# lisanhu/LongReadMapper

Hardware: AMD Instinct MI355X
Metric: aligned Gbp/sec (higher is better)
Workload: dtype u8/u64 integer; 1 GPU; E. coli K-12 sized synthetic reference (4641652 bp, 5% planted repeats), 100000 x 10000 bp ont-profile reads per GPU; seed_len=20, thres=300, gact_T=320, gact_O=120, gact_W=128, reads_per_gpu=100000, read_len=10000, streams=3, sa_sampled=1, parallelism=reads sharded, index replicated (1 RCCL bcast)

## Files before the change

### longreadmapper_amd/csrc/index_tables.hip

```cpp
#include <hip/hip_runtime.h>
#include <cstdio>
#include "seed_index_dev.h"

__device__ __forceinline__ uint64_t lcl_entry(const LrmIndexView &ix, int hl, uint64_t code) {
    const int ext = hl - ix.hlen;
    uint64_t k, l;
    lc_lookup(ix, code >> (2 * ext), k, l);
    if (k == 0 && l == 0) return 0;
    for (int i = ext - 1; i >= 0 && k <= l; --i) {
        const uint32_t c = (uint32_t) (code >> (2 * i)) & 3u;
        uint64_t ra, rb;
        occ_lf2(ix, c, k - 1, l, ra, rb);
        k = ra + 1;
        l = rb;
    }
    if (k > l) return 0;
    const uint64_t cnt = l - k + 1;
    return cnt >= 0xFFFFFFull ? (0xFFFFFFull << 40) : (k | (cnt << 40));
}

__global__ __launch_bounds__(256) void lcl_build_kernel(LrmIndexView ix, int hl, int pair, int kbits, uint64_t *__restrict__ out,
                                                        uint64_t slot0, uint64_t *__restrict__ ovf, uint64_t ovf_cap,
                                                        unsigned long long *__restrict__ n_ovf) {
    const uint64_t slot = slot0 + (uint64_t) blockIdx.x * 256 + threadIdx.x;
// ... 92 lines not shown
    }
    bool to_side = rr >= cmax;
    for (uint32_t r = 0; r < (uint32_t) sdv.sd_f; ++r) {
        const SdKey key = sd_key_of(sdv, code, r);
        uint64_t *line = sd + key.line * 8;
        bool placed = false;
        if (sdv.sd_slot == 8) {
            const uint64_t v = k | (c << sdv.sd_kbits) | (key.tag << (64u - key.tb));
            for (int sl = 0; sl < 8 && !placed; ++sl)
                placed = atomicCAS((unsigned long long *) &line[sl], 0ull, (unsigned long long) v) == 0ull;
            if (!placed) atomicOr((unsigned long long *) &line[0], 1ull << (63u - key.tb));
        } else {
            const uint64_t v = k | (c << sdv.sd_kbits) | (key.tag << (48u - key.tb));
            const uint32_t at = atomicAdd(reinterpret_cast<uint32_t *>(line) + 15, 1u) & 0xFFu;
            if (at >= 250u) atomicAdd(n_ovf, 1ull << 40);
            if (at >= 10u) atomicOr(reinterpret_cast<uint32_t *>(line) + 15, 1u << (8u + sd_filter_bit((uint32_t) key.tag)));
            if (at < 10u) {
                uint16_t *h = reinterpret_cast<uint16_t *>(line) + 3 * at;
                h[0] = (uint16_t) v; h[1] = (uint16_t) (v >> 16); h[2] = (uint16_t) (v >> 32);
                placed = true;
            }
        }
        if (!placed) to_side = true;
    }
    if (to_side) {
        const unsigned long long at = atomicAdd(n_ovf, 1ull);
        if (at < ovf_cap) { ovf[2 * at] = code; ovf[2 * at + 1] = side; }
    }
}

__global__ __launch_bounds__(256) void sd_clear_kernel(ulonglong2 *__restrict__ p, uint64_t n16) {
    for (uint64_t i = (uint64_t) blockIdx.x * 256 + threadIdx.x; i < n16; i += (uint64_t) gridDim.x * 256) p[i] = make_ulonglong2(0, 0);
}

struct SdPlan { int f, bits, slot, kbits, cbits; uint64_t bytes; };
static bool sd_plan(const lrm_index *idx, uint64_t free_b, SdPlan *pl) {
    const LrmIndexTune &tu = idx->itune;
    const uint64_t L = idx->view.length;
    const int S = tu.sd_len;
    if (tu.sd == 0 || !idx->cpl_ok || L < 64 || idx->view.con_len != L) return false;
    int kbits = 1;
    while ((1ull << kbits) < L) ++kbits;
    for (int f = 4; f >= 2; f -= 2) {
        if (tu.sd_f && tu.sd_f != f) continue;
        const int slot = f == 4 ? 8 : 6, lf = f == 4 ? 2 : 1;
        const double target = f == 4 ? 2.2 : 6.0;
        int bits = 10;
        while ((double) f * (double) L / (double) (1ull << bits) > target && bits < 34) ++bits;
        if (tu.sd_bits) bits = tu.sd_bits;
        const int CL2 = 2 * (S - f + 1);
        if (bits > CL2) bits = CL2;
        if (bits < 11) bits = 11;
        if (bits < CL2 - 31) bits = CL2 - 31;
        const int tb = lf + 2 * (f - 1) + (CL2 - bits);
        int cbits = (slot == 8 ? 63 : 48) - tb - kbits;
        if (cbits < (tu.sd_bits ? 2 : 4) || tb > 40) continue;
        if (cbits > 24) cbits = 24;
        if (tu.sd_cbits && tu.sd_cbits < cbits) cbits = tu.sd_cbits;
        const uint64_t bytes = 64ull << bits;
        const uint64_t spare = bytes >= (32ull << 30) ? (40ull << 30) : (8ull << 30);
        if (tu.sd < 0 && ((uint64_t) free_b < bytes + bytes / 8 + spare || (tu.lc_long_max >= 13 && bytes > (16ull << 30)))) continue;
        pl->f = f; pl->bits = bits; pl->slot = slot; pl->kbits = kbits; pl->cbits = cbits; pl->bytes = bytes;
        return true;
    }
    return false;
}
static void sd_filter_build(lrm_index *idx);
static int sd_build(lrm_index *idx, const SdPlan &pl) {
    uint64_t *d = nullptr, *ovf = nullptr, *tab = nullptr;
    uint32_t *claimed = nullptr;
    unsigned long long *n_ovf = nullptr;
    const char *why = "";
    unsigned long long n = 0;
    auto give_up = [&]() {
        if (idx->mtune.verbose) fprintf(stderr, "[lrm] seed table (share %d, 2^%d lines, %d-byte slots) not built: %s (side entries %llu)\n", pl.f, pl.bits, pl.slot, why, n);
        if (d) (void) hipFree(d); if (ovf) (void) hipFree(ovf); if (tab) (void) hipFree(tab); if (n_ovf) (void) hipFree(n_ovf);
        if (claimed) (void) hipFree(claimed);
        (void) hipGetLastError(); return 0; };
    const uint64_t L = idx->view.length, lines = 1ull << pl.bits;
    uint64_t ovf_cap = lines / 4 + 4096;
    if (ovf_cap > (1ull << 30)) ovf_cap = 1ull << 30;
    if (idx->itune.sd_bits) ovf_cap = (uint64_t) pl.f * L + 4096;
    why = "no room for the table";
    if (hipMalloc(&d, pl.bytes) != hipSuccess) { d = nullptr; return give_up(); }
    why = "no room for the overflow list";
    if (hipMalloc(&ovf, ovf_cap * 16) != hipSuccess) { ovf = nullptr; return give_up(); }
    if (hipMalloc(&n_ovf, 8) != hipSuccess) { n_ovf = nullptr; return give_up(); }
    const uint64_t cl_bytes = ((L + 31) / 32 + 1) * 4;
    if (hipMalloc(&claimed, cl_bytes) != hipSuccess) { claimed = nullptr; return give_up(); }
    why = "memset failed";
    if (hipMemset(claimed, 0, cl_bytes) != hipSuccess) return give_up();
    hipLaunchKernelGGL(sd_clear_kernel, dim3(256 * 64), dim3(256), 0, 0, reinterpret_cast<ulonglong2 *>(d), pl.bytes / 16);
    if (hipGetLastError() != hipSuccess || hipMemset(n_ovf, 0, 8) != hipSuccess) return give_up();
    LrmIndexView sdv = idx->view;
    sdv.sd_len = idx->itune.sd_len; sdv.sd_f = pl.f; sdv.sd_bits = pl.bits; sdv.sd_kbits = pl.kbits; sdv.sd_slot = pl.slot; sdv.sd_cbits = pl.cbits;
    const uint64_t chunk = 1ull << 22;
    for (uint64_t b0 = 0, blocks = (L + 255) / 256; b0 < blocks; b0 += chunk) {
        const uint64_t nb = blocks - b0 < chunk ? blocks - b0 : chunk;
        hipLaunchKernelGGL(sd_build_kernel, dim3((uint32_t) nb), dim3(256), 0, 0, idx->view, sdv, d, b0 * 256, claimed, ovf, ovf_cap, n_ovf);
    }
    why = "build kernel failed";
    if (hipDeviceSynchronize() != hipSuccess) { give_up(); lrm_set_error("seed table build failed"); return -1; }
    why = "too many entries beside their lines";
    if (hipMemcpy(&n, n_ovf, 8, hipMemcpyDeviceToHost) != hipSuccess || n > ovf_cap) return give_up();
    uint64_t tslots = 1024;
    while (tslots < 2 * n) tslots <<= 1;
    why = "no room for the side table";
    if (hipMalloc(&tab, tslots * 16) != hipSuccess) { tab = nullptr; return give_up(); }
    if (hipMemset(tab, 0, tslots * 16) != hipSuccess) return give_up();
    if (n) hipLaunchKernelGGL(lclx_build_kernel, dim3((uint32_t) ((n + 255) / 256)), dim3(256), 0, 0, ovf, (uint64_t) n, tab, tslots - 1);
    if (hipDeviceSynchronize() != hipSuccess) { give_up(); lrm_set_error("seed table side build failed"); return -1; }
    (void) hipFree(ovf); (void) hipFree(n_ovf); (void) hipFree(claimed);
    idx->d_sd = d; idx->d_sdx = tab;
    idx->view.sd = d; idx->view.sdx = tab; idx->view.sdx_mask = tslots - 1;
    idx->view.sd_len = sdv.sd_len; idx->view.sd_f = pl.f; idx->view.sd_bits = pl.bits; idx->view.sd_kbits = pl.kbits; idx->view.sd_slot = pl.slot;
    idx->view.sd_cbits = pl.cbits;
    idx->sd_side_entries = n;
    if (idx->mtune.verbose) fprintf(stderr, "[lrm] seed table: %d positions per line, 2^%d lines, %d-byte slots, %d count bits, %llu side entries\n", pl.f, pl.bits, pl.slot, pl.cbits, n);
    sd_filter_build(idx);
    return 0;
}

__global__ __launch_bounds__(256) void sd_filter_kernel(const ulonglong2 *__restrict__ sd, uint64_t lines, uint32_t g,
                                                        uint32_t *__restrict__ filt) {
    const uint64_t line = (uint64_t) blockIdx.x * 256 + threadIdx.x;
    if (line >= lines) return;
    const ulonglong2 x0 = sd[line * 4], x1 = sd[line * 4 + 1], x2 = sd[line * 4 + 2], x3 = sd[line * 4 + 3];
    if (((x0.x | x0.y) | (x1.x | x1.y) | (x2.x | x2.y) | (x3.x | x3.y)) == 0) return;
    const uint64_t bit = line >> g;
    const uint32_t m = 1u << (bit & 31u);
    if (!(filt[bit >> 5] & m)) atomicOr(&filt[bit >> 5], m);
}
__global__ __launch_bounds__(256) void sd_filter_count_kernel(const uint32_t *__restrict__ filt, uint64_t words,
                                                              unsigned long long *__restrict__ n_set) {
    uint32_t c = 0;
    for (uint64_t i = (uint64_t) blockIdx.x * 256 + threadIdx.x; i < words; i += (uint64_t) gridDim.x * 256) c += __popc(filt[i]);
    for (int o = 32; o > 0; o >>= 1) c += __shfl_down(c, o, 64);
    if ((threadIdx.x & 63u) == 0 && c) atomicAdd(n_set, (unsigned long long) c);
}
static void sd_filter_build(lrm_index *idx) {
    const LrmIndexView &v = idx->view;
    const int kb = idx->itune.sd_filter_kb;
    if (kb <= 0 || !lrm_sd48_form(v)) return;
    const uint64_t lines = 1ull << v.sd_bits, max_bits = (uint64_t) kb * 8192;
    uint32_t g = 0;
    while ((lines >> g) > max_bits) ++g;
    const uint64_t bits = lines >> g;
    if (bits < 512) return;
    if ((double) v.length / (double) bits > 4.0 * 0.6931471805599453) {
        if (idx->mtune.verbose) fprintf(stderr, "[lrm] seed filter: not built, %.1f rows per bit at %d KiB\n", (double) v.length / (double) bits, kb);
        return;
    }
    uint32_t *filt = nullptr;
    unsigned long long *d_n = nullptr, n_set = 0;
    bool ok = hipMalloc(&filt, bits / 8 + 64) == hipSuccess && hipMalloc(&d_n, 8) == hipSuccess
              && hipMemset(filt, 0, bits / 8 + 64) == hipSuccess && hipMemset(d_n, 0, 8) == hipSuccess;
    if (ok) {
        const uint64_t chunk = 1ull << 30;
        for (uint64_t l0 = 0; l0 < lines; l0 += chunk) {
            const uint64_t nl = lines - l0 < chunk ? lines - l0 : chunk;
            hipLaunchKernelGGL(sd_filter_kernel, dim3((uint32_t) ((nl + 255) / 256)), dim3(256), 0, 0,
                               reinterpret_cast<const ulonglong2 *>(v.sd) + l0 * 4, nl, g, filt + ((l0 >> g) >> 5));
        }
        hipLaunchKernelGGL(sd_filter_count_kernel, dim3(256), dim3(256), 0, 0, filt, bits / 32, d_n);
        ok = hipDeviceSynchronize() == hipSuccess && hipMemcpy(&n_set, d_n, 8, hipMemcpyDeviceToHost) == hipSuccess;
    }
    if (d_n) (void) hipFree(d_n);
    const bool keep = ok && 2 * n_set <= bits;
    if (idx->mtune.verbose && ok)
        fprintf(stderr, "[lrm] seed filter: %llu bytes, one bit per %u lines, %.1f %% of the bits set%s\n", (unsigned long long) (bits / 8), 1u << g,
                100.0 * (double) n_set / (double) bits, keep ? "" : ": more than half, not kept");
    if (!keep) { if (filt) (void) hipFree(filt); (void) hipGetLastError(); return; }
    idx->d_sd_filt = filt;
    idx->view.sd_filt = filt; idx->view.sd_filt_shift = (int32_t) g;
}
// ... 91 lines not shown
```

### longreadmapper_amd/csrc/lrm_internal.h

```cpp
#pragma once
#include <stddef.h>
#include <stdint.h>
#include <stdlib.h>
#include <string.h>
#include "../../include/lrm_accel.h"

#define LRM_BLOB_MAGIC 0x4c524d424c4f4232ull
#define LRM_OCC_ROWS 64

struct LrmOccEntry {
    uint64_t cnt;
    uint64_t mask;
};
struct LrmOccBlock { LrmOccEntry sym[4]; };
static_assert(sizeof(LrmOccBlock) == 64, "occ block must be one 64-B line");

struct LrmMtaDev { uint64_t offset, seq_len; };

struct LrmBlobHeader {
    uint64_t magic, version;
    uint64_t length;
    uint64_t c4[4];
    uint64_t dollar_row;
    uint64_t n_blocks;
    uint64_t lc_entries;
    uint64_t sa_len, con_len;
    uint64_t off_occ, off_lc, off_sa, off_content, off_mta;
    uint64_t total_bytes;
    int32_t hlen, mta_len;
    uint64_t off_lcx, n_lcx;
    uint64_t sa_ratio;
    uint64_t reserved[10];
};
static_assert(sizeof(LrmBlobHeader) == 256, "header is 256 B");

struct LrmIndexView {
    const LrmOccBlock *occ;
    const uint64_t *lc;
    const uint64_t *lcx;
    uint64_t n_lcx;
    const uint64_t *sa;
    const char *content;
    const LrmMtaDev *mta;
    uint64_t length, dollar_row, sa_len, con_len;
    uint64_t c4[4];
    int32_t hlen, mta_len;
    const uint64_t *lcl;
    int32_t hl;
    int32_t sa_shift;
    int32_t lcl_pair;
    int32_t lcl_kbits;
    const uint64_t *core;
    const uint64_t *lclx;
    uint64_t lclx_mask;
    const uint64_t *sd;
    const uint64_t *sdx;
    uint64_t sdx_mask;
    int32_t sd_len;
    int32_t sd_f;
    int32_t sd_bits;
    int32_t sd_kbits;
    int32_t sd_slot;
    int32_t sd_cbits;
    const uint32_t *sd_filt;
    int32_t sd_filt_shift;
};
static inline bool lrm_sd48_form(const LrmIndexView &v) {
    return v.sd && v.sd_f == 4 && v.sd_slot == 8 && 8 + 2 * (v.sd_len - 3) - v.sd_bits <= 32;
}

struct LrmEnv {
    static constexpr int MAXV = 32;
    const char *name[MAXV];
    long long val[MAXV];
    int n;
    bool get(const char *key, long long *out) const;
};
void lrm_env_snapshot(LrmEnv *e);
#define LRM_SD_FILTER_KB_DEFAULT 4096
struct LrmIndexTune {
    int sa_ratio;
    int lc_long, lc_long_max, lc_pair, lc_entry_bytes, lc_count_bits, lc_core;
    int sd, sd_len, sd_f, sd_bits, sd_cbits;
    int sd_filter_kb;
    uint64_t lcx_threshold;
};
struct LrmMapTune {
    int dense, gact_impl, seed_rounds, cigar_text, keep_reads, anchored;
    uint32_t anchor_min_len;
    uint32_t clip, clip_penalty, clip_end_bonus;
    uint32_t split, split_min_len;
    uint32_t slice_reads, sub_batches, group_subs, bs_waves, copy_threads;
    uint32_t ss_items, ss_lds_pad, vote_vg, vote_t1, vote_u, vote_load, vote_fast;
    uint32_t t3_limit, t3_slots;
    int ext_streams, seed_streams, verbose;
};
void lrm_resolve_index_tune(const lrm_index_options *opt, const LrmEnv &env, LrmIndexTune *out);
void lrm_resolve_map_tune(const lrm_map_options *opt, const LrmEnv &env, LrmMapTune *out);
template <typename T>
static inline void lrm_options_over_defaults(T *o, const T *opt) {
    if (opt) memcpy(o, opt, opt->struct_size && opt->struct_size < sizeof(T) ? opt->struct_size : sizeof(T));
}
template <typename T>
static inline void lrm_options_take_fields(T *o, const T *opt, size_t from, size_t to) {
    if (opt && opt->struct_size >= to) memcpy((char *) o + from, (const char *) opt + from, to - from);
}

struct LrmHostCtx;
struct lrm_index;
void lrm_call_map_tune(const lrm_index *ix, const lrm_map_options *opt, LrmMapTune *out);
struct lrm_index {
    void *d_blob;
    uint64_t blob_bytes;
    int owns_blob;
    int device;
    LrmBlobHeader hdr;
    LrmIndexView view;
    uint64_t *d_lcl;
    uint64_t *d_lclx;
    uint64_t *d_core;
    uint64_t *d_sd, *d_sdx;
    uint64_t sd_side_entries;
    uint32_t *d_sd_filt;
    uint64_t *d_cpl;
    int cpl_ok;
    uint64_t *d_sas;
    LrmHostCtx *host;
    int n_peers;
    lrm_index **peers;
    LrmEnv env;
    LrmIndexTune itune;
    LrmMapTune mtune;
    uint32_t dbg_t3_limit, dbg_t3_slots;
    uint32_t dbg_mapq_slots;
};

struct LrmPhaseRes {
    uint64_t key1, val1, bucket1;
    uint64_t key2, val2, bucket2;
};

struct LrmDevCounters {
    unsigned long long bs_queue;
    unsigned long long vote_ticket[2];
    unsigned long long seed_traffic[3];
    unsigned long long reserved[2];
    unsigned long long decided_phase0;
    unsigned long long gact_tiles;
    unsigned long long pad[2];
    unsigned long long vote_fast_ticket[2];
    unsigned long long vote_redo_n[2];
    unsigned long long vote_big_n[2];
// ... 176 lines not shown
```

### longreadmapper_amd/csrc/seed_index_dev.h

```cpp
#pragma once
#include "lrm_hip_util.h"

__device__ __forceinline__ uint32_t base_code(uint32_t c) { return ((c >> 1) ^ (c >> 2)) & 3u; }

__device__ __forceinline__ uint32_t occ_lf2(const LrmIndexView &ix, uint32_t c, uint64_t loc_a, uint64_t loc_b,
                                            uint64_t &ra, uint64_t &rb) {
    const ulonglong2 eb = *reinterpret_cast<const ulonglong2 *>(&ix.occ[loc_b >> 6].sym[c]);
    ulonglong2 ea = eb;
    const bool two = (loc_a >> 6) != (loc_b >> 6);
    if (two) ea = *reinterpret_cast<const ulonglong2 *>(&ix.occ[loc_a >> 6].sym[c]);
    ra = occ_lf_of(ea, loc_a);
    rb = occ_lf_of(eb, loc_b);
    return two ? 2u : 1u;
}

__device__ __forceinline__ void lc_lookup(const LrmIndexView &ix, uint64_t code, uint64_t &k, uint64_t &l) {
    const uint64_t e = ix.lc[code];
    k = e & ((1ull << 40) - 1ull);
    const uint64_t cnt = e >> 40;
    l = k + cnt - 1;
    if (e == 0) { k = 0; l = 0; }
    else if (cnt == 0xFFFFFFull) {
        uint64_t lo = 0, hi = ix.n_lcx;
        while (lo < hi) { uint64_t mid = (lo + hi) >> 1; if (ix.lcx[3 * mid] < code) lo = mid + 1; else hi = mid; }
        k = ix.lcx[3 * lo + 1];
        l = ix.lcx[3 * lo + 2];
    }
}

struct SdKey { uint64_t line; uint64_t tag; uint32_t tb; };
__device__ __forceinline__ SdKey sd_key_of(const LrmIndexView &ix, uint64_t code, uint32_t r) {
    const uint32_t lf = ix.sd_f == 4 ? 2u : 1u, F = 1u << lf, lo_n = F - 1u - r;
    const uint32_t CL2 = 2u * ((uint32_t) ix.sd_len - F + 1u), wlo = CL2 < 32u ? CL2 : 32u;
    const uint64_t core = (code >> (2u * lo_n)) & ((1ull << CL2) - 1ull);
    const uint32_t extra = (uint32_t) (code & ((1ull << (2u * lo_n)) - 1ull)) | ((uint32_t) (code >> (2u * lo_n + CL2)) << (2u * lo_n));
    uint32_t m = (uint32_t) core * 0x9E3779B1u;
    if (wlo < 32u) m &= (1u << wlo) - 1u;
    const uint32_t chi = ((uint32_t) (core >> 32) ^ m) & ((1u << (CL2 - wlo)) - 1u);
    const uint32_t rb = CL2 - (uint32_t) ix.sd_bits;
    SdKey key;
    key.line = ((uint64_t) chi << (wlo - rb)) | (uint64_t) (m >> rb);
    key.tb = lf + 2u * (F - 1u) + rb;
    key.tag = (uint64_t) (r | (extra << lf)) | ((uint64_t) (m & ((1u << rb) - 1u)) << (lf + 2u * (F - 1u)));
    return key;
}
__device__ __forceinline__ uint32_t sd_filter_bit(uint32_t tag) { return (((tag * 0x9E3779B1u) >> 27) * 24u) >> 5; }
__device__ __forceinline__ bool sd_side_lookup(const LrmIndexView &ix, uint64_t code, uint64_t &e) {
    uint64_t slot = (code * 0x9E3779B97F4A7C15ull) >> 20 & ix.sdx_mask;
    for (;;) {
        const ulonglong2 x = *reinterpret_cast<const ulonglong2 *>(ix.sdx + 2 * slot);
        if (x.x == code + 1) { e = x.y; return true; }
        if (x.x == 0) return false;
        slot = (slot + 1) & ix.sdx_mask;
    }
}
__device__ __forceinline__ int sd_search(const LrmIndexView &ix, const SdKey &key, uint64_t code, const uint64_t (&W)[8],
                                         uint64_t &k, uint64_t &c, uint32_t *cnt) {
    uint64_t e = 0;
    bool ovf;
    if (ix.sd_slot == 8) {
        if (key.tb <= 32u) {
            const uint32_t sh = 32u - key.tb, t32 = (uint32_t) key.tag;
            uint32_t elo = 0, ehi = 0;
#pragma unroll
            for (int i = 7; i >= 0; --i) {
                const uint32_t hi = (uint32_t) (W[i] >> 32);
                const bool m = (hi >> sh) == t32;
                elo = m ? (uint32_t) W[i] : elo;
                ehi = m ? hi : ehi;
            }
            e = (uint64_t) elo | ((uint64_t) ehi << 32);
        } else {
#pragma unroll
            for (int i = 7; i >= 0; --i)
                if ((W[i] >> (64u - key.tb)) == key.tag) e = W[i];
        }
        ovf = (W[0] >> (63u - key.tb)) & 1ull;
    } else {
        uint32_t D[16];
#pragma unroll
        for (int i = 0; i < 8; ++i) { D[2 * i] = (uint32_t) W[i]; D[2 * i + 1] = (uint32_t) (W[i] >> 32); }
        if (key.tb <= 16u) {
            const uint32_t sh = 16u - key.tb, t32 = (uint32_t) key.tag;
            uint32_t elo = 0, ehi = 0;
#pragma unroll
            for (int i = 9; i >= 0; --i) {
                const int h2 = 3 * i + 2;
                const uint32_t hw = (h2 & 1) ? D[h2 >> 1] >> 16 : D[h2 >> 1] & 0xFFFFu;
                const uint32_t lo = (i & 1) ? __builtin_amdgcn_alignbit(D[(3 * i + 1) >> 1], D[(3 * i) >> 1], 16) : D[(3 * i) >> 1];
                const bool m = (hw >> sh) == t32;
                elo = m ? lo : elo;
                ehi = m ? hw : ehi;
            }
            e = (uint64_t) elo | ((uint64_t) ehi << 32);
        } else {
#pragma unroll
            for (int i = 9; i >= 0; --i) {
                const int w = (48 * i) >> 6, off = (48 * i) & 63;
                uint64_t v = W[w] >> off;
                if (off > 16) v |= W[w + 1] << (64 - off);
                v &= (1ull << 48) - 1ull;
                if ((v >> (48u - key.tb)) == key.tag) e = v;
            }
        }
        ovf = (D[15] & 0xFFu) > 10u && ((D[15] >> (8u + sd_filter_bit((uint32_t) key.tag))) & 1u);
    }
    const uint64_t cmax = (1ull << ix.sd_cbits) - 1ull;
    if (e != 0) {
        k = e & ((1ull << ix.sd_kbits) - 1ull);
        c = (e >> ix.sd_kbits) & cmax;
        if (c == 0) { k |= LRM_LOCATED_BIT; c = 1; return 1; }
        if (c != cmax) return 1;
    } else if (!ovf) {
        return 0;
    }
    uint64_t se;
    if (cnt) cnt[0] += 2;
    if (!sd_side_lookup(ix, code, se)) return e != 0 ? 2 : 0;
    if ((se >> 40) == 0xFFFFFFull) return 2;
    k = se & ((1ull << 40) - 1ull);
    c = se >> 40;
    return 1;
}
__device__ __forceinline__ int sd_lookup(const LrmIndexView &ix, uint64_t win, uint32_t jpar, uint64_t &k, uint64_t &c, uint32_t *cnt) {
    const uint64_t code = win & ((1ull << (2 * ix.sd_len)) - 1ull);
    const SdKey key = sd_key_of(ix, code, jpar & (uint32_t) (ix.sd_f - 1));
    const uint64_t *line = ix.sd + key.line * 8;
    const ulonglong2 x0 = *reinterpret_cast<const ulonglong2 *>(line), x1 = *reinterpret_cast<const ulonglong2 *>(line + 2);
    const ulonglong2 x2 = *reinterpret_cast<const ulonglong2 *>(line + 4), x3 = *reinterpret_cast<const ulonglong2 *>(line + 6);
    if (cnt) cnt[0] += 1;
    const uint64_t W[8] = {x0.x, x0.y, x1.x, x1.y, x2.x, x2.y, x3.x, x3.y};
    return sd_search(ix, key, code, W, k, c, cnt);
}

__device__ __forceinline__ uint64_t seed_one(const LrmIndexView &ix, uint64_t win, int seed_len, uint32_t jpar,
                                             uint64_t &k, uint64_t &l, uint32_t *cnt = nullptr) {
    int left = seed_len - ix.hlen;
    bool looked_up = false;
    if (ix.sd && seed_len == ix.sd_len) {
        uint64_t c;
        const int st = sd_lookup(ix, win, jpar, k, c, cnt);
        if (st == 0) { k = 0; l = 0; return 0; }
        if (st == 1) { l = k + c - 1; return c; }
    }
    if (ix.core && seed_len >= 16) {
        const int left2 = seed_len - 16;
        const uint64_t W = (win >> (2 * left2)) & 0xFFFFFFFFull;
        const uint32_t r = jpar & 3u;
        const uint64_t corec = (W >> (2 * (3 - r))) & ((1ull << 26) - 1ull);
        const uint32_t extra = (uint32_t) (W & ((1ull << (2 * (3 - r))) - 1ull)) | ((uint32_t) (W >> (2 * (16 - r))) << (2 * (3 - r)));
        const uint32_t tag = r | (extra << 2);
        const uint64_t *line = ix.core + corec * 8;
        const ulonglong2 x0 = *reinterpret_cast<const ulonglong2 *>(line), x1 = *reinterpret_cast<const ulonglong2 *>(line + 2);
        const ulonglong2 x2 = *reinterpret_cast<const ulonglong2 *>(line + 4), x3 = *reinterpret_cast<const ulonglong2 *>(line + 6);
        if (cnt) cnt[0] += 1;
        const uint64_t sl[8] = {x0.x, x0.y, x1.x, x1.y, x2.x, x2.y, x3.x, x3.y};
        uint64_t e = 0;
        int state = x0.x == ~0ull ? 3 : 2;
#pragma unroll
        for (int i = 0; i < 8; ++i)
            if (sl[i] != 0 && sl[i] != ~0ull && (uint32_t) (sl[i] >> 56) == tag) { e = sl[i]; state = 1; }
        if (state != 3) {
            if (state != 1) { k = 0; l = 0; return 0; }
            k = e & ((1ull << 40) - 1ull);
            l = k + ((e >> 40) & 0xFFFFull) - 1;
            left = left2;
            looked_up = true;
        }
    }
    if (!looked_up && ix.lcl && seed_len >= ix.hl) {
        const int left2 = seed_len - ix.hl;
        uint64_t at = (win >> (2 * left2)) & ((1ull << (2 * ix.hl)) - 1ull);
        if (ix.lcl_pair) {
            const uint64_t smask = (1ull << (2 * (ix.hl - 1))) - 1ull;
            at = (jpar & 1u) ? ((at & smask) << 3) + 4u + (at >> (2 * (ix.hl - 1)))
                             : ((at >> 2) << 3) + (at & 3u);
        }
        uint64_t e;
        if (ix.lcl_kbits) {
            uint64_t v;
            __builtin_memcpy(&v, reinterpret_cast<const uint8_t *>(ix.lcl) + at * 5, 8);
            v &= (1ull << 40) - 1ull;
            const uint64_t c5 = v >> ix.lcl_kbits, cmax = (1ull << (40 - ix.lcl_kbits)) - 1ull;
            e = v == 0 ? 0ull : (v & ((1ull << ix.lcl_kbits) - 1ull)) | (c5 << 40);
            if (c5 == cmax) {
                const uint64_t code = (win >> (2 * left2)) & ((1ull << (2 * ix.hl)) - 1ull);
                uint64_t slot = (code * 0x9E3779B97F4A7C15ull) >> 20 & ix.lclx_mask;
                for (;;) {
                    const ulonglong2 x = *reinterpret_cast<const ulonglong2 *>(ix.lclx + 2 * slot);
// ... 40 lines not shown
```

### longreadmapper_amd/csrc/seed_kernels.hip

```cpp
#include <hip/hip_runtime.h>
#include "seed_index_dev.h"

__global__ __launch_bounds__(256) void pack2bit_kernel(const char *__restrict__ reads, uint64_t stride,
                                                       const uint32_t *__restrict__ lens,
                                                       uint8_t *__restrict__ out, uint64_t bytes_per_read,
                                                       uint32_t chunks_per_read, uint64_t n) {
    uint64_t read = blockIdx.x / chunks_per_read;
    uint32_t chunk = blockIdx.x % chunks_per_read;
    if (read >= n) return;
    uint64_t ow = (uint64_t) chunk * 256 + threadIdx.x;
    if (ow * 4 >= bytes_per_read) return;
    uint32_t len = lens[read];
    const uint8_t *r = (const uint8_t *) reads + read * stride;
    uint64_t p = ow * 16;
    uint32_t v = 0;
    if (p + 16 <= len) {
        uint32_t w[4];
        __builtin_memcpy(w, r + p, 16);
#pragma unroll
        for (int t = 0; t < 16; ++t) v |= base_code((w[t >> 2] >> (8 * (t & 3))) & 0xffu) << (2 * t);
    } else {
        for (int t = 0; t < 16; ++t) {
            uint32_t code = (p + t < len) ? base_code(r[p + t]) : 0u;
            v |= code << (2 * t);
        }
    }
    *reinterpret_cast<uint32_t *>(out + read * bytes_per_read + ow * 4) = v;
}

template <int CTRL>
__device__ __forceinline__ uint64_t quad_perm64(uint64_t v) {
    const uint32_t lo = (uint32_t) __builtin_amdgcn_update_dpp(0, (int) (uint32_t) v, CTRL, 0xf, 0xf, true);
    const uint32_t hi = (uint32_t) __builtin_amdgcn_update_dpp(0, (int) (uint32_t) (v >> 32), CTRL, 0xf, 0xf, true);
    return (uint64_t) lo | ((uint64_t) hi << 32);
}
__device__ __forceinline__ void sd_issue_shared(const LrmIndexView &ix, const SdKey &key, ulonglong2 &a, ulonglong2 &b) {
    const uint32_t lane = __lane_id();
    if (ix.sd_f == 4) {
        const uint64_t line = quad_perm64<0x00>(key.line);
        a = *reinterpret_cast<const ulonglong2 *>(ix.sd + line * 8 + (lane & 3u) * 2);
        b = a;
    } else {
        const uint64_t line = quad_perm64<0xA0>(key.line);
        const uint64_t *src = ix.sd + line * 8 + (lane & 1u) * 4;
        a = *reinterpret_cast<const ulonglong2 *>(src);
        b = *reinterpret_cast<const ulonglong2 *>(src + 2);
    }
}
__device__ __forceinline__ uint32_t sd_filter_issue(const LrmIndexView &ix, const SdKey &key, bool real, uint32_t &bit) {
    const uint64_t line = quad_perm64<0x00>(key.line);
    bit = real ? (uint32_t) (line >> (uint32_t) ix.sd_filt_shift) : 0u;
    return ix.sd_filt[bit >> 5];
}
__device__ __forceinline__ void sd_issue_filtered(const LrmIndexView &ix, const SdKey &key, bool real, uint32_t word, uint32_t bit,
                                                  ulonglong2 &a, ulonglong2 &b) {
    const uint32_t lane = __lane_id();
    const uint64_t line = quad_perm64<0x00>(key.line);
    const uint64_t *zeros = reinterpret_cast<const uint64_t *>(ix.sd_filt + ((1ull << ix.sd_bits) >> (uint32_t) ix.sd_filt_shift >> 5));
    const bool pass = real && ((word >> (bit & 31u)) & 1u);
    const uint64_t *src = pass ? ix.sd + line * 8 : zeros;
    a = *reinterpret_cast<const ulonglong2 *>(src + (lane & 3u) * 2);
    b = a;
}
__device__ __forceinline__ int sd_finish_shared(const LrmIndexView &ix, const SdKey &key, uint64_t code, const ulonglong2 &a, const ulonglong2 &b,
                                                uint64_t &k, uint64_t &c, uint32_t *cnt) {
    uint64_t W[8];
    if (ix.sd_f == 4) {
        W[0] = quad_perm64<0x00>(a.x); W[1] = quad_perm64<0x00>(a.y);
        W[2] = quad_perm64<0x55>(a.x); W[3] = quad_perm64<0x55>(a.y);
        W[4] = quad_perm64<0xAA>(a.x); W[5] = quad_perm64<0xAA>(a.y);
        W[6] = quad_perm64<0xFF>(a.x); W[7] = quad_perm64<0xFF>(a.y);
    } else {
        const uint64_t pa = quad_perm64<0xB1>(a.x), pb = quad_perm64<0xB1>(a.y);
        const uint64_t pc = quad_perm64<0xB1>(b.x), pd = quad_perm64<0xB1>(b.y);
        const bool odd = __lane_id() & 1u;
        W[0] = odd ? pa : a.x; W[1] = odd ? pb : a.y; W[2] = odd ? pc : b.x; W[3] = odd ? pd : b.y;
        W[4] = odd ? a.x : pa; W[5] = odd ? a.y : pb; W[6] = odd ? b.x : pc; W[7] = odd ? b.y : pd;
    }
    if (cnt) cnt[0] += 1;
    return sd_search(ix, key, code, W, k, c, cnt);
}

struct __attribute__((aligned(8))) WordPair { uint64_t a, b; };

__device__ __forceinline__ uint64_t read_window(const uint64_t *__restrict__ words, uint32_t j) {
    uint32_t wi = j >> 5, sh = (j & 31) * 2;
    WordPair w;
    __builtin_memcpy(&w, words + wi, sizeof(w));
    return (w.a >> sh) | ((w.b << 1) << (63 - sh));
}

__device__ __forceinline__ void ss_append(uint64_t *s_tot, uint64_t *s_rec, uint32_t *s_q, uint32_t cap_pp, uint32_t ph, uint32_t q, uint64_t k,
                                          uint64_t rr) {
    const uint32_t slot = (uint32_t) atomicAdd(reinterpret_cast<unsigned long long *>(&s_tot[ph]), 1ull | (rr << 32));
    s_rec[ph * cap_pp + slot] = k | (rr << 40);
    s_q[ph * cap_pp + slot] = q;
}

template <int SS_ITEMS, bool COUNT, bool SD48, bool FILT = false>
__global__ __launch_bounds__(256) __attribute__((amdgpu_waves_per_eu(COUNT ? 1 : 6, 8)))
void seed_search_kernel(LrmIndexView ix, const uint64_t *__restrict__ reads2,
                                                          uint64_t words_per_read,
                                                          const uint32_t *__restrict__ lens,
                                                          const uint8_t *__restrict__ decided, uint64_t n,
                                                          int seed_len, uint32_t thres, int phase_lo, int phase_hi,
                                                          uint32_t cap_q, uint32_t blocks_per_read,
                                                          uint64_t *__restrict__ rec, uint32_t *__restrict__ recq,
                                                          uint32_t *__restrict__ gcnt, uint32_t *__restrict__ ghits,
                                                          LrmDevCounters *counters) {
    __shared__ uint64_t s_rec[SS_ITEMS + 64];
    __shared__ uint32_t s_traffic[3];
    uint32_t my_cnt[2] = {0, 0}, my_seeds = 0;
    if (COUNT && threadIdx.x < 3) s_traffic[threadIdx.x] = 0;
    __shared__ uint32_t s_q[SS_ITEMS + 64];
    __shared__ uint64_t s_tot[64];
    __shared__ uint32_t s_base[64];
    const uint64_t read = blockIdx.x / blocks_per_read;
    const uint32_t chunk = blockIdx.x % blocks_per_read;
    if (read >= n) return;
    if (decided && decided[read]) return;
    const int P = seed_len + 1;
    const uint32_t np = (uint32_t) (phase_hi - phase_lo + 1);
    const uint32_t cap_pp = SS_ITEMS / np + 1;
    const uint32_t tid = threadIdx.x;
    if (tid < np) s_tot[tid] = 0;
    __syncthreads();
    const uint32_t len = lens[read];
    const uint32_t jl = len > (uint32_t) seed_len ? len - (uint32_t) seed_len : 0;
    const uint64_t *words = reads2 + read * words_per_read;
    const bool dense_lanes = (uint32_t) P - np <= 1u;
    const bool shared_lines = ix.sd && seed_len == ix.sd_len && np == (uint32_t) P && phase_lo == 0;
    LrmIndexView ix_nosd = ix;
    ix_nosd.sd = nullptr;
    LrmIndexView ixs = ix;
    if (SD48) { ixs.sd_f = 4; ixs.sd_slot = 8; }
    if (shared_lines) {
        const uint32_t lim = jl < cap_q * np ? jl : cap_q * np;
        const uint32_t np_inv = 0xFFFFFFFFu / np;
        const uint64_t smask = (1ull << (2 * seed_len)) - 1ull;
        const uint32_t dq = 256u / np, dph = 256u % np;
        uint32_t q = __umulhi(chunk * SS_ITEMS + tid, np_inv), ph = chunk * SS_ITEMS + tid - q * np;
        if (ph >= np) { ++q; ph -= np; }
        if (ph >= np) { ++q; ph -= np; }
        struct Look { uint64_t code; SdKey key; ulonglong2 a, b; bool have, real; uint32_t word, bit; };
        auto look = [&](bool real, uint32_t j, uint32_t j0) {
            Look f;
            f.have = real && j < lim;
            f.code = 0;
            f.key.line = 0; f.key.tag = 0; f.key.tb = 0;
            if (real) {
                const uint64_t *wp = words + (j0 >> 5);
                const uint64_t W0 = wp[0], W1 = wp[1], W2 = wp[2];
                const uint32_t rel = j - j0, sh = (rel & 31u) * 2u;
                const uint64_t lo = rel < 32u ? W0 : W1, hi = rel < 32u ? W1 : W2;
                f.code = f.have ? ((lo >> sh) | ((hi << 1) << (63 - sh))) & smask : 0ull;
                f.key = sd_key_of(ixs, f.code, j & (uint32_t) (ixs.sd_f - 1));
            }
            if (SD48) __builtin_assume(f.key.tb <= 32u);
            f.real = real;
            if (FILT) f.word = sd_filter_issue(ixs, f.key, real, f.bit);
            else sd_issue_shared(ixs, f.key, f.a, f.b);
            if (SD48) __builtin_amdgcn_sched_barrier(0);
            return f;
        };
        uint32_t j = chunk * SS_ITEMS + tid;
        uint32_t j0 = (uint32_t) __builtin_amdgcn_readfirstlane((int) (j & ~63u));
        auto take = [&](const Look &f) {
            uint64_t k = 0, l = 0, c = 0, rr;
            const int st = sd_finish_shared(ixs, f.key, f.code, f.a, f.b, k, c, COUNT ? my_cnt : nullptr);
            if (f.have) {
                if (st == 1) rr = c;
                else if (st == 0) rr = 0;
                else rr = seed_one(ix_nosd, f.code, seed_len, j, k, l, COUNT ? my_cnt : nullptr);
                if (COUNT) my_seeds++;
                if (rr > 0 && rr < (uint64_t) thres) ss_append(s_tot, s_rec, s_q, cap_pp, ph, q, k, rr);
            }
        };
        auto step = [&]() {
            j += 256u; j0 += 256u;
            q += dq; ph += dph;
            if (ph >= np) { ++q; ph -= np; }
        };
        if (j0 < lim) {
            const uint32_t left = (lim - j0 + 255u) >> 8;
            const uint32_t n_it = left < (uint32_t) (SS_ITEMS / 256) ? left : (uint32_t) (SS_ITEMS / 256);
            if (FILT) {
                auto fetch = [&](Look f) {
                    sd_issue_filtered(ixs, f.key, f.real, f.word, f.bit, f.a, f.b);
                    __builtin_amdgcn_sched_barrier(0);
                    return f;
                };
                Look pa = look(true, j, j0), pb = look(1 < n_it, j + 256u, j0 + 256u);
                Look ga = fetch(pa), gb;
                uint32_t it = 0;
#pragma unroll 1
                do {
                    pa = look(it + 2 < n_it, j + 512u, j0 + 512u);
                    gb = fetch(pb);
                    take(ga);
                    step();
                    pb = look(it + 3 < n_it, j + 512u, j0 + 512u);
                    ga = fetch(pa);
                    if (it + 1 < n_it) take(gb);
                    step();
                    it += 2;
                } while (it < n_it);
            } else if (SD48) {
                Look fa = look(true, j, j0), fb;
                uint32_t it = 0;
#pragma unroll 1
                do {
                    fb = look(it + 1 < n_it, j + 256u, j0 + 256u);
                    take(fa);
                    step();
                    fa = look(it + 2 < n_it, j + 256u, j0 + 256u);
                    if (it + 1 < n_it) take(fb);
                    step();
                    it += 2;
                } while (it < n_it);
            } else {
#pragma unroll 1
                for (uint32_t it = 0; it < n_it; ++it) {
                    const Look f = look(true, j, j0);
                    take(f);
                    step();
                }
            }
        }
    } else {
    const uint32_t np_inv_g = 0xFFFFFFFFu / np;
#pragma unroll 1
    for (uint32_t it = 0; it < SS_ITEMS / 256; ++it) {
        const uint32_t item = chunk * SS_ITEMS + it * 256 + tid;
        uint32_t q = __umulhi(item, np_inv_g), ph = item - q * np;
        if (ph >= np) { ++q; ph -= np; }
        if (ph >= np) { ++q; ph -= np; }
        uint64_t W[6] = {0, 0, 0, 0, 0, 0};
        uint32_t jw = 0;
        if (dense_lanes) {
            const uint32_t item0 = (uint32_t) __builtin_amdgcn_readfirstlane((int) (item & ~63u));
            const uint32_t q0 = item0 / np;
            if (q0 < cap_q) {
                const uint32_t j0 = (uint32_t) phase_lo + item0 % np + q0 * (uint32_t) P;
                const uint64_t *wp = words + (j0 >> 5);
                jw = j0 & ~31u;
#pragma unroll
                for (int e = 0; e < 6; ++e) W[e] = wp[e];
            }
        }
        if (q >= cap_q) break;
        const uint32_t j = (uint32_t) phase_lo + ph + q * (uint32_t) P;
        if (j >= jl) continue;
        uint64_t win, k, l;
        if (dense_lanes) {
            const uint32_t rel = j - jw, wi = rel >> 5, sh = (rel & 31u) * 2u;
            const uint64_t lo = wi == 0 ? W[0] : wi == 1 ? W[1] : wi == 2 ? W[2] : wi == 3 ? W[3] : W[4];
            const uint64_t hi = wi == 0 ? W[1] : wi == 1 ? W[2] : wi == 2 ? W[3] : wi == 3 ? W[4] : W[5];
            win = (lo >> sh) | ((hi << 1) << (63 - sh));
        } else {
            win = read_window(words, j);
        }
        const uint64_t rr = seed_one(ix, win, seed_len, j, k, l, COUNT ? my_cnt : nullptr);
        if (COUNT) my_seeds++;
        if (rr > 0 && rr < (uint64_t) thres) ss_append(s_tot, s_rec, s_q, cap_pp, ph, q, k, rr);
    }
    }
    if (COUNT) { atomicAdd(&s_traffic[0], my_seeds); atomicAdd(&s_traffic[1], my_cnt[0]); atomicAdd(&s_traffic[2], my_cnt[1]); }
    __syncthreads();
    if (COUNT && tid < 3) atomicAdd(&counters->seed_traffic[tid], (unsigned long long) s_traffic[tid]);
    if (tid < np) {
        const uint64_t tot = s_tot[tid];
// ... 78 lines not shown
            LrmPhaseRes r = pr[iter];
            uint64_t v = r.val1 + r.val2;
            if (5 * v > 3 * num_seeds) {
                out.key = r.key1; out.val = r.val1; out.bucket = r.bucket1;
                if (mode == 2 && iter == 0 && P > 1) atomicAdd(&counters->decided_phase0, 1ull);
                break;
            } else if (r.val1 != 0) {
                uint64_t key = r.key1, bucket = key >> 4;
                bool found = false;
                for (int t = 0; t < ot_n; ++t) {
                    if (ot_bucket[t] == bucket) {
                        found = true;
                        ot_val[t] += 1;
                        if (key < ot_key[t]) ot_key[t] = key;
                    }
                }
                if (!found) { ot_key[ot_n] = key; ot_val[ot_n] = 1; ot_bucket[ot_n] = bucket; ot_n++; }
            }
        }
    }
    if (iter >= P - 1) {
        lrm_entry t1 = {0, 0, 0};
        for (int t = 0; t < ot_n; ++t)
            if (t1.val < ot_val[t]) { t1.key = ot_key[t]; t1.val = ot_val[t]; t1.bucket = ot_bucket[t]; }
        out = t1;
    }
    best[read] = out;
    if (phase_out) phase_out[read] = (uint8_t) (iter < P ? iter : P - 1);
}


int lrm_launch_seed(lrm_index *idx, lrm_workspace *ws, const char *d_reads, uint64_t stride,
                    const uint32_t *d_lens, uint64_t n, uint32_t seed_len,
                    uint32_t thres, lrm_entry *d_best, const LrmMapTune &mt, void *stream_, uint8_t *d_phase_out) {
    hipStream_t stream = (hipStream_t) stream_;
    if (n == 0) return 0;
    ws->seeded_best = nullptr; ws->seeded_n = 0; ws->seeded_phase = 0;
    const int P = (int) seed_len + 1;
    const uint32_t cap_q = ws->cap_q;
    const uint64_t wpr = ws->words_per_read;

    HIPCHK(hipMemsetAsync(ws->d_counters, 0, sizeof(LrmDevCounters), stream));
    HIPCHK(hipMemsetAsync(ws->d_hcount, 0, n * (uint64_t) P * 4, stream));
    HIPCHK(hipMemsetAsync(ws->d_cnt, 0, n * (uint64_t) P * 4, stream));
    ws->n_last = n;
    {
        uint64_t bpr = wpr * 8;
        uint32_t cpr = (uint32_t) ((bpr / 4 + 255) / 256);
        uint32_t grid;
        if (lrm_grid_1d(n * cpr, "pack2bit", &grid)) return -1;
        lrm_time_begin(ws, LRM_K_PACK2BIT, stream);
        hipLaunchKernelGGL(pack2bit_kernel, dim3(grid), dim3(256), 0, stream, d_reads, stride,
                           d_lens, (uint8_t *) ws->d_reads2, bpr, cpr, n);
        lrm_time_end(ws, stream);
    }
    uint32_t tbits = 1;
    while ((1u << tbits) < thres && tbits < 31) tbits++;
    if (((uint64_t) cap_q << tbits) > 0xffffffffull) {
        lrm_set_error("read too long for the vote order key: cap_q %u << %u bits exceeds 32 bits", cap_q, tbits);
        return -1;
    }
    bool single = false;
    {
        const volatile uint64_t *hist = reinterpret_cast<const volatile uint64_t *>(ws->h_err + 2);
        const uint64_t d0 = *hist;
        if (ws->hist_n >= 64 && d0 * 50 < ws->hist_n) single = true;
        if (mt.seed_rounds == 1 || mt.seed_rounds == 2) single = mt.seed_rounds == 1;
        if (P == 1) single = true;
    }
    for (int round = single ? 1 : 0; round < 2; ++round) {
        int lo = round == 0 || single ? 0 : 1;
        int hi = round == 0 ? 0 : P - 1;
        if (lo > hi) break;
        int np = hi - lo + 1;
        const uint8_t *dec = round == 0 || single ? nullptr : ws->d_decided;
        const uint32_t ss_items = mt.ss_items;
        uint32_t bpr = (uint32_t) (((uint64_t) np * cap_q + ss_items - 1) / ss_items);
        uint32_t grid;
        if (lrm_grid_1d(n * bpr, "seed_search", &grid)) return -1;
        lrm_time_begin(ws, LRM_K_SEED_SEARCH, stream);
        const LrmIndexView &v = idx->view;
        const bool sd48 = lrm_sd48_form(v);
        const bool filt = sd48 && v.sd_filt;
        auto sk = ws->counting ? seed_search_kernel<2048, true, false>
                  : filt ? (ss_items == 1024u ? seed_search_kernel<1024, false, true, true> : ss_items == 4096u ? seed_search_kernel<4096, false, true, true> : seed_search_kernel<2048, false, true, true>)
                  : sd48 ? (ss_items == 1024u ? seed_search_kernel<1024, false, true> : ss_items == 4096u ? seed_search_kernel<4096, false, true> : seed_search_kernel<2048, false, true>)
                         : (ss_items == 1024u ? seed_search_kernel<1024, false, false> : ss_items == 4096u ? seed_search_kernel<4096, false, false> : seed_search_kernel<2048, false, false>);
        if (ws->counting) bpr = (uint32_t) (((uint64_t) np * cap_q + 2047) / 2048);
        if (ws->counting) grid = (uint32_t) (n * bpr);
        hipLaunchKernelGGL(sk, dim3(grid), dim3(256), mt.ss_lds_pad, stream, idx->view,
                           ws->d_reads2, wpr, d_lens, dec, n, (int) seed_len, thres, lo, hi, cap_q, bpr,
                           ws->d_rec, ws->d_recq, ws->d_cnt, ws->d_hcount, ws->d_counters);
        lrm_time_end(ws, stream);
        const LrmVoteLaunch vl = {dec, n, seed_len, lo, hi, tbits, round, &mt};
        if (lrm_launch_vote(idx, ws, vl, stream)) return -1;
        lrm_time_begin(ws, LRM_K_DECIDE, stream);
        hipLaunchKernelGGL(decide_kernel, dim3((uint32_t) ((n + 255) / 256)), dim3(256), 0, stream, ws->d_phase,
                           d_lens, n, (int) seed_len, single ? 2 : round, ws->d_decided, d_best, ws->d_counters, d_phase_out);
        lrm_time_end(ws, stream);
    }
    HIPCHK(hipMemcpyAsync((void *) (ws->h_err + 2), &ws->d_counters->decided_phase0, 8, hipMemcpyDeviceToHost, stream));
    ws->hist_n = n;
    HIPCHK(hipGetLastError());
    ws->seeded_best = d_best; ws->seeded_n = n;
    ws->seeded_phase = d_phase_out != nullptr && d_phase_out == ws->d_mq_phase;
    return 0;
}

int lrm_launch_debug_seed(lrm_index *idx, const char *d_read, uint32_t len, uint32_t seed_len,
                          uint64_t *d_reads2, uint64_t words, int32_t *d_j, uint64_t *d_rr,
                          uint64_t *d_k, uint64_t *d_l, uint64_t cap, void *stream_) {
    hipStream_t stream = (hipStream_t) stream_;
    const uint32_t P = seed_len + 1;
    uint32_t jl = len > seed_len ? len - seed_len : 0;
    uint32_t cap_q = (jl + P - 1) / P;
    if (cap_q == 0) cap_q = 1;
    if ((uint64_t) cap_q * P > cap) { lrm_set_error("debug seed buffer too small"); return -1; }
    uint64_t bpr = words * 8;
    uint32_t cpr = (uint32_t) ((bpr / 4 + 255) / 256);
    uint32_t *d_len1 = (uint32_t *) (d_reads2 + words);
    HIPCHK(hipMemcpyAsync(d_len1, &len, sizeof(uint32_t), hipMemcpyHostToDevice, stream));
    hipLaunchKernelGGL(pack2bit_kernel, dim3(cpr), dim3(256), 0, stream, d_read, (uint64_t) 0, d_len1,
                       (uint8_t *) d_reads2, bpr, cpr, (uint64_t) 1);
    uint32_t items = cap_q * P;
    hipLaunchKernelGGL(seed_search_debug_kernel, dim3((items + 255) / 256), dim3(256), 0, stream, idx->view,
                       d_reads2, len, (int) seed_len, cap_q, d_j, d_rr, d_k, d_l);
    HIPCHK(hipGetLastError());
    return (int) cap_q;
}
```

Baseline: 66.79 Gbp/s.

## Add 32-bit offset seed-table probe path with DPP quad slot scan

Adds an OFF32 variant of the filtered seed search kernel, used when the seed table has at most 2^25 lines. It computes byte offsets in 32 bits, redirects filtered-out lookups to a zeroed tail region appended to the table, and scans each quad's slots with 32-bit DPP broadcasts instead of building a 64-bit shared word array. It also simplifies code extraction per lane. The aim is to cut VGPR pressure and 64-bit address arithmetic in the hot probe loop, at the cost of another kernel instantiation and a small padded tail allocation.

```diff
diff --git a/longreadmapper_amd/csrc/index_tables.hip b/longreadmapper_amd/csrc/index_tables.hip
--- a/longreadmapper_amd/csrc/index_tables.hip
+++ b/longreadmapper_amd/csrc/index_tables.hip
@@ -198,7 +198,7 @@
     if (ovf_cap > (1ull << 30)) ovf_cap = 1ull << 30;
     if (idx->itune.sd_bits) ovf_cap = (uint64_t) pl.f * L + 4096;
     why = "no room for the table";
-    if (hipMalloc(&d, pl.bytes) != hipSuccess) { d = nullptr; return give_up(); }
+    if (hipMalloc(&d, pl.bytes + LRM_SD_TAIL) != hipSuccess) { d = nullptr; return give_up(); }
     why = "no room for the overflow list";
     if (hipMalloc(&ovf, ovf_cap * 16) != hipSuccess) { ovf = nullptr; return give_up(); }
     if (hipMalloc(&n_ovf, 8) != hipSuccess) { n_ovf = nullptr; return give_up(); }
@@ -206,7 +206,7 @@
     if (hipMalloc(&claimed, cl_bytes) != hipSuccess) { claimed = nullptr; return give_up(); }
     why = "memset failed";
     if (hipMemset(claimed, 0, cl_bytes) != hipSuccess) return give_up();
-    hipLaunchKernelGGL(sd_clear_kernel, dim3(256 * 64), dim3(256), 0, 0, reinterpret_cast<ulonglong2 *>(d), pl.bytes / 16);
+    hipLaunchKernelGGL(sd_clear_kernel, dim3(256 * 64), dim3(256), 0, 0, reinterpret_cast<ulonglong2 *>(d), (pl.bytes + LRM_SD_TAIL) / 16);
     if (hipGetLastError() != hipSuccess || hipMemset(n_ovf, 0, 8) != hipSuccess) return give_up();
     LrmIndexView sdv = idx->view;
     sdv.sd_len = idx->itune.sd_len; sdv.sd_f = pl.f; sdv.sd_bits = pl.bits; sdv.sd_kbits = pl.kbits; sdv.sd_slot = pl.slot; sdv.sd_cbits = pl.cbits;
diff --git a/longreadmapper_amd/csrc/lrm_internal.h b/longreadmapper_amd/csrc/lrm_internal.h
--- a/longreadmapper_amd/csrc/lrm_internal.h
+++ b/longreadmapper_amd/csrc/lrm_internal.h
@@ -68,6 +68,8 @@
 static inline bool lrm_sd48_form(const LrmIndexView &v) {
     return v.sd && v.sd_f == 4 && v.sd_slot == 8 && 8 + 2 * (v.sd_len - 3) - v.sd_bits <= 32;
 }
+#define LRM_SD_TAIL 64
+static inline bool lrm_sd_off32(const LrmIndexView &v) { return v.sd_bits <= 25; }
 
 struct LrmEnv {
     static constexpr int MAXV = 32;
diff --git a/longreadmapper_amd/csrc/seed_index_dev.h b/longreadmapper_amd/csrc/seed_index_dev.h
--- a/longreadmapper_amd/csrc/seed_index_dev.h
+++ b/longreadmapper_amd/csrc/seed_index_dev.h
@@ -54,6 +54,7 @@
         slot = (slot + 1) & ix.sdx_mask;
     }
 }
+__device__ __forceinline__ int sd_answer(const LrmIndexView &ix, uint64_t code, uint64_t e, bool ovf, uint64_t &k, uint64_t &c, uint32_t *cnt);
 __device__ __forceinline__ int sd_search(const LrmIndexView &ix, const SdKey &key, uint64_t code, const uint64_t (&W)[8],
                                          uint64_t &k, uint64_t &c, uint32_t *cnt) {
     uint64_t e = 0;
@@ -105,6 +106,9 @@
         }
         ovf = (D[15] & 0xFFu) > 10u && ((D[15] >> (8u + sd_filter_bit((uint32_t) key.tag))) & 1u);
     }
+    return sd_answer(ix, code, e, ovf, k, c, cnt);
+}
+__device__ __forceinline__ int sd_answer(const LrmIndexView &ix, uint64_t code, uint64_t e, bool ovf, uint64_t &k, uint64_t &c, uint32_t *cnt) {
     const uint64_t cmax = (1ull << ix.sd_cbits) - 1ull;
     if (e != 0) {
         k = e & ((1ull << ix.sd_kbits) - 1ull);
diff --git a/longreadmapper_amd/csrc/seed_kernels.hip b/longreadmapper_amd/csrc/seed_kernels.hip
--- a/longreadmapper_amd/csrc/seed_kernels.hip
+++ b/longreadmapper_amd/csrc/seed_kernels.hip
@@ -62,6 +62,38 @@
     a = *reinterpret_cast<const ulonglong2 *>(src + (lane & 3u) * 2);
     b = a;
 }
+__device__ __forceinline__ uint32_t sd_filter_issue32(const LrmIndexView &ix, const SdKey &key, uint32_t &bit, uint32_t &line) {
+    line = (uint32_t) __builtin_amdgcn_update_dpp(0, (int) (uint32_t) key.line, 0x00, 0xf, 0xf, true);
+    bit = line >> (uint32_t) ix.sd_filt_shift;
+    return ix.sd_filt[bit >> 5];
+}
+__device__ __forceinline__ void sd_issue_filtered32(const LrmIndexView &ix, bool real, uint32_t word, uint32_t bit, uint32_t line,
+                                                    uint32_t piece, uint32_t zpiece, ulonglong2 &a, ulonglong2 &b) {
+    const bool pass = real && ((word >> (bit & 31u)) & 1u);
+    const uint32_t off = pass ? (line << 6) + piece : zpiece;
+    a = *reinterpret_cast<const ulonglong2 *>(reinterpret_cast<const char *>(ix.sd) + off);
+    b = a;
+}
+template <int CTRL>
+__device__ __forceinline__ void sd_slot32(uint64_t w, uint32_t tsh, uint32_t lim, uint32_t &elo, uint32_t &ex, uint32_t &x, uint32_t &lo) {
+    x = (uint32_t) __builtin_amdgcn_update_dpp(0, (int) (uint32_t) (w >> 32), CTRL, 0xf, 0xf, true) ^ tsh;
+    lo = (uint32_t) __builtin_amdgcn_update_dpp(0, (int) (uint32_t) w, CTRL, 0xf, 0xf, true);
+    const bool m = x < lim;
+    elo = m ? lo : elo;
+    ex = m ? x : ex;
+}
+__device__ __forceinline__ int sd_finish_quad32(const LrmIndexView &ix, const SdKey &key, uint64_t code, const ulonglong2 &a,
+                                                uint64_t &k, uint64_t &c) {
+    const uint32_t sh = 32u - key.tb, tsh = (uint32_t) key.tag << sh;
+    uint32_t lim = 1u << sh, elo = 0, ex = tsh, x, lo;
+    asm("" : "+s"(lim));
+    sd_slot32<0xFF>(a.y, tsh, lim, elo, ex, x, lo); sd_slot32<0xFF>(a.x, tsh, lim, elo, ex, x, lo);
+    sd_slot32<0xAA>(a.y, tsh, lim, elo, ex, x, lo); sd_slot32<0xAA>(a.x, tsh, lim, elo, ex, x, lo);
+    sd_slot32<0x55>(a.y, tsh, lim, elo, ex, x, lo); sd_slot32<0x55>(a.x, tsh, lim, elo, ex, x, lo);
+    sd_slot32<0x00>(a.y, tsh, lim, elo, ex, x, lo); sd_slot32<0x00>(a.x, tsh, lim, elo, ex, x, lo);
+    const bool ovf = key.tb == 32u ? lo >> 31 : (x >> (sh - 1u)) & 1u;
+    return sd_answer(ix, code, (uint64_t) elo | ((uint64_t) (ex ^ tsh) << 32), ovf, k, c, nullptr);
+}
 __device__ __forceinline__ int sd_finish_shared(const LrmIndexView &ix, const SdKey &key, uint64_t code, const ulonglong2 &a, const ulonglong2 &b,
                                                 uint64_t &k, uint64_t &c, uint32_t *cnt) {
     uint64_t W[8];
@@ -97,7 +129,7 @@
     s_q[ph * cap_pp + slot] = q;
 }
 
-template <int SS_ITEMS, bool COUNT, bool SD48, bool FILT = false>
+template <int SS_ITEMS, bool COUNT, bool SD48, bool FILT = false, bool OFF32 = false>
 __global__ __launch_bounds__(256) __attribute__((amdgpu_waves_per_eu(COUNT ? 1 : 6, 8)))
 void seed_search_kernel(LrmIndexView ix, const uint64_t *__restrict__ reads2,
                                                           uint64_t words_per_read,
@@ -142,7 +174,8 @@
         uint32_t q = __umulhi(chunk * SS_ITEMS + tid, np_inv), ph = chunk * SS_ITEMS + tid - q * np;
         if (ph >= np) { ++q; ph -= np; }
         if (ph >= np) { ++q; ph -= np; }
-        struct Look { uint64_t code; SdKey key; ulonglong2 a, b; bool have, real; uint32_t word, bit; };
+        const uint32_t lane_rel = tid & 63u;
+        struct Look { uint64_t code; SdKey key; ulonglong2 a, b; bool have, real; uint32_t word, bit, line; };
         auto look = [&](bool real, uint32_t j, uint32_t j0) {
             Look f;
             f.have = real && j < lim;
@@ -151,14 +184,21 @@
             if (real) {
                 const uint64_t *wp = words + (j0 >> 5);
                 const uint64_t W0 = wp[0], W1 = wp[1], W2 = wp[2];
+                if (OFF32) {
+                    const uint32_t sh = (lane_rel & 31u) * 2u;
+                    const uint64_t c0 = (W0 >> sh) | ((W1 << 1) << (63 - sh)), c1 = (W1 >> sh) | ((W2 << 1) << (63 - sh));
+                    f.code = f.have ? (lane_rel < 32u ? c0 : c1) & smask : 0ull;
+                } else {
                 const uint32_t rel = j - j0, sh = (rel & 31u) * 2u;
                 const uint64_t lo = rel < 32u ? W0 : W1, hi = rel < 32u ? W1 : W2;
                 f.code = f.have ? ((lo >> sh) | ((hi << 1) << (63 - sh))) & smask : 0ull;
+                }
                 f.key = sd_key_of(ixs, f.code, j & (uint32_t) (ixs.sd_f - 1));
             }
             if (SD48) __builtin_assume(f.key.tb <= 32u);
             f.real = real;
-            if (FILT) f.word = sd_filter_issue(ixs, f.key, real, f.bit);
+            if (FILT && OFF32) f.word = sd_filter_issue32(ixs, f.key, f.bit, f.line);
+            else if (FILT) f.word = sd_filter_issue(ixs, f.key, real, f.bit);
             else sd_issue_shared(ixs, f.key, f.a, f.b);
             if (SD48) __builtin_amdgcn_sched_barrier(0);
             return f;
@@ -167,7 +207,8 @@
         uint32_t j0 = (uint32_t) __builtin_amdgcn_readfirstlane((int) (j & ~63u));
         auto take = [&](const Look &f) {
             uint64_t k = 0, l = 0, c = 0, rr;
-            const int st = sd_finish_shared(ixs, f.key, f.code, f.a, f.b, k, c, COUNT ? my_cnt : nullptr);
+            const int st = OFF32 ? sd_finish_quad32(ixs, f.key, f.code, f.a, k, c)
+                                 : sd_finish_shared(ixs, f.key, f.code, f.a, f.b, k, c, COUNT ? my_cnt : nullptr);
             if (f.have) {
                 if (st == 1) rr = c;
                 else if (st == 0) rr = 0;
@@ -185,8 +226,11 @@
             const uint32_t left = (lim - j0 + 255u) >> 8;
             const uint32_t n_it = left < (uint32_t) (SS_ITEMS / 256) ? left : (uint32_t) (SS_ITEMS / 256);
             if (FILT) {
+                uint32_t piece = (tid & 3u) * 16u, zpiece = (64u << ixs.sd_bits) + piece;
+                if (OFF32) asm volatile("" : "+v"(piece), "+v"(zpiece));
                 auto fetch = [&](Look f) {
-                    sd_issue_filtered(ixs, f.key, f.real, f.word, f.bit, f.a, f.b);
+                    if (OFF32) sd_issue_filtered32(ixs, f.real, f.word, f.bit, f.line, piece, zpiece, f.a, f.b);
+                    else sd_issue_filtered(ixs, f.key, f.real, f.word, f.bit, f.a, f.b);
                     __builtin_amdgcn_sched_barrier(0);
                     return f;
                 };
@@ -431,7 +475,9 @@
         const LrmIndexView &v = idx->view;
         const bool sd48 = lrm_sd48_form(v);
         const bool filt = sd48 && v.sd_filt;
+        const bool off32 = filt && lrm_sd_off32(v);
         auto sk = ws->counting ? seed_search_kernel<2048, true, false>
+                  : off32 ? (ss_items == 1024u ? seed_search_kernel<1024, false, true, true, true> : ss_items == 4096u ? seed_search_kernel<4096, false, true, true, true> : seed_search_kernel<2048, false, true, true, true>)
                   : filt ? (ss_items == 1024u ? seed_search_kernel<1024, false, true, true> : ss_items == 4096u ? seed_search_kernel<4096, false, true, true> : seed_search_kernel<2048, false, true, true>)
                   : sd48 ? (ss_items == 1024u ? seed_search_kernel<1024, false, true> : ss_items == 4096u ? seed_search_kernel<4096, false, true> : seed_search_kernel<2048, false, true>)
                          : (ss_items == 1024u ? seed_search_kernel<1024, false, false> : ss_items == 4096u ? seed_search_kernel<4096, false, false> : seed_search_kernel<2048, false, false>);
```

Result: faster. 67.47 Gbp/s, median of 6 (+1.0%).
